# waveygang/wfmash

Measured on AMD Instinct MI355X. Metric: aligned bases/sec (whole node) + CIGAR-identical rate vs CPU ref, higher is better.
Workload: dtype int32; 1 GPU; C3: 64 synthetic 5%-divergence 50kb segment pairs per GPU, WFA-only (BiWFA gap-affine-2p 5,8,2,24,1; mappings pre-supplied); pairs_per_gpu=64, pairs_total=64, parallelism=records sharded over 1 GPU(s)

## Files before the change

wfmash_amd/csrc/wfa_device.h:

```cpp
#ifndef WFM_WFA_DEVICE_H_
#define WFM_WFA_DEVICE_H_

#include <hip/hip_runtime.h>
#include <stdint.h>

#include "wfa_rows.h"

namespace wfm {

constexpr int WF_NULL = -(1 << 30);
constexpr int RING = 32;
constexpr int RMASK = RING - 1;
constexpr int RING_BIG = 128;

enum { C_M = 0, C_I1 = 1, C_I2 = 2, C_D1 = 3, C_D2 = 4 };
enum { OP_M = 0, OP_X = 1, OP_I = 2, OP_D = 3 };
enum { BT_I1_EXT = 8, BT_I2_EXT = 16, BT_D1_EXT = 32, BT_D2_EXT = 64 };

constexpr int WFM_DEV_UNREACHABLE = -300;
constexpr int WFM_DEV_OVERFLOW = -2;
constexpr int WFM_DEV_BAND = -4;
constexpr int WFM_DEV_P2_NOTHING = -6;
constexpr int WFM_DEV_LIMIT = -7;
constexpr int WFM_DEV_P2_MORE = -5;
// ... 79 lines not shown
  int32_t score, score_fwd, score_rev, k_fwd, off_fwd, comp;
  int32_t steps;
  uint64_t cells;
  int32_t steps_p1;
  uint32_t ticks_p1, ticks_p2;
  int32_t pad_;
  uint32_t ticks_list, ticks_pick;
  uint32_t work_items, pad2_;
};

struct BaseJob {
  int64_t p_off, t_off;
  int64_t pre_off;
  int64_t bt_off;
  int64_t ring_off;
  int64_t rle_end;
  int32_t pl, tl;
  int32_t comp_begin, comp_end;
  int32_t endsfree, pbf, pef, tbf, tef;
  int32_t smax, kmin, width;
  int32_t type;
  int32_t pad_;
  int32_t score_only;
};
static_assert(sizeof(BaseJob) == 112, "BaseJob::score_only fills the struct's tail padding: the job arrays keep their stride");

struct BaseResult {
  int32_t status;
  int32_t score;
  int32_t nruns;
  int32_t pad_;
  uint64_t cells;
};

struct Base2TJob {
  BaseJob b;
  int64_t snap_in, snap_out;
  int32_t ntiles, core;
  int32_t task0;
  int32_t s0;
  int32_t done;
  int32_t end_s, end_k, end_off;
};
struct Base2TTask { int32_t job, tile; };
constexpr int B2T_ROWS = 32;
constexpr int B2T_THREADS = 512;
void launch_base2t_block(const uint32_t* pk, int32_t* a32, uint8_t* a8, const Base2TJob* jobs, const Base2TTask* tasks, unsigned long long* tile_key,
                         int32_t* tile_off, int ntasks, int T, hipStream_t st);
void launch_base2t_advance(Base2TJob* jobs, const unsigned long long* tile_key, const int32_t* tile_off, int njobs, int T, int32_t* active_slot, hipStream_t st);
void launch_base2t_finish(const int32_t* a32, const uint8_t* a8, uint32_t* rle, const Base2TJob* jobs, BaseResult* res, int njobs, hipStream_t st);

struct BoundJob { int64_t p_off, t_off; int32_t pl, tl; };
void launch_bound(const uint8_t* seq, const BoundJob* jobs, int32_t* out, int njobs, DevPen pen, hipStream_t st);

struct SeqRev { int64_t p_fwd, p_rev, t_fwd, t_rev; int32_t plen, tlen; };
void launch_reverse(uint8_t* seq, const SeqRev* jobs, int njobs, int pad, hipStream_t st);
struct SeqGatherTask { const uint8_t* src; uint8_t* dst; int32_t len, pad; int32_t reverse, complement; };
void launch_seq_gather(const SeqGatherTask* tasks, int64_t ntasks, hipStream_t st);
struct CheckProb {
  int64_t p_off, t_off;
  uint64_t run_off;
  uint32_t n_runs;
  int32_t plen, tlen;
  int32_t pbf, pef, tbf, tef;
  int32_t res_score;
  uint32_t res_ops_len;
  int32_t skip;
};
struct CheckTask { int32_t prob, slice; };
void launch_check(const uint8_t* seq, const uint32_t* runs, const CheckProb* probs, int nprob, const CheckTask* tasks, int64_t ntasks,
                  uint32_t* ops_pre, uint32_t* p_pre, uint32_t* t_pre, uint32_t* cmp_ops, unsigned long long* keys, void* out, DevPen pen,
                  hipStream_t st);
struct OptProb {
  int64_t p_off, t_off, row_off;
  int32_t plen, tlen;
  int32_t pbf, pef, tbf, tef;
  int32_t band_lo, band_hi;
};
void launch_optcheck(const uint8_t* seq, const OptProb* probs, int nprob, int form, int32_t* rows, int32_t* out, DevPen pen, hipStream_t st);
void launch_seq_normalize(uint8_t* seq, int64_t nbytes, hipStream_t st);
void launch_seq_pack(const uint8_t* seq, uint32_t* pk, int64_t nwords, int64_t nbytes, const SeqRev* jobs, int njobs, int32_t* flag, hipStream_t st);
constexpr int64_t PK_PAD_WORDS = 2048 + 64;
void launch_tile2(const uint32_t* pk, int32_t* ring, const TileJob* jobs, const TileTask* tasks, int32_t* mak, int ntasks, int threads, int T, int variants, hipStream_t st);
bool tile2_coarse_maxima();
void launch_tile2_p2(const uint32_t* pk, int32_t* ring, const TileJob* jobs, const TileTask* tasks, int ntasks, int threads, int32_t* p2, hipStream_t st);
int selftest_dpp(int* host_out128, hipStream_t st);
void launch_base2(const uint32_t* pk, int32_t* a32, uint8_t* a8, uint32_t* rle, const BaseJob* jobs, BaseResult* res, int njobs, int threads, hipStream_t st);
void launch_bp(const uint8_t* seq, int32_t* ring, const BpJob* jobs, BpResult* res, int njobs, int threads,
               DevPen pen, int scope, int ring_rows, hipStream_t st);
void launch_tile_init(const uint8_t* seq, int32_t* ring, const TileJob* jobs, int32_t* mak0, int njobs, int ring_rows, hipStream_t st);
void launch_tile(const uint8_t* seq, int32_t* ring, const TileJob* jobs, const TileTask* tasks, int32_t* mak, int ntasks,
                 int threads, int T, int Wt, size_t lds_bytes, DevPen pen, int scope, int ring_rows, hipStream_t st);
void launch_tile_advance(TileJob* jobs, int32_t* mak, int njobs, int T, DevPen pen, int exact, int coarse, int launched, hipStream_t st);
void launch_tile_reg(const uint8_t* seq, int32_t* ring, const TileJob* jobs, const TileTask* tasks, int32_t* mak, int ntasks,
                     int threads, int T, int C, bool cut, hipStream_t st);
void launch_tile_p2(const uint8_t* seq, int32_t* ring, const TileJob* jobs, const TileTask* tasks, int ntasks, int threads,
                    int32_t* p2, bool cut, hipStream_t st);
void launch_p2_to_ring(int32_t* ring, const int32_t* p2, const P2Job* jobs, int njobs, hipStream_t st);
struct RingWidenJob {
  const int32_t* src;
  int32_t* dst;
  int32_t src_w, src_koff;
  int32_t dst_w, dst_koff;
  int32_t klo, khi;
};
void launch_ring_widen(const RingWidenJob* jobs, int njobs, int max_dst_w, int ring_rows, hipStream_t st);
void launch_p2_blockmax(const int32_t* ring, const int32_t* p2, const P2Job* jobs, int32_t* bmax, int32_t* p2max, int njobs, hipStream_t st);
void launch_p2_overlap(const int32_t* ring, const int32_t* p2, const P2Job* jobs, const int32_t* p2max, const int32_t* bmax, int32_t* pbmax,
                       BpResult* res, int njobs, int threads, int max_nblk, DevPen pen, int scope, hipStream_t st);
void launch_base(const uint8_t* seq, int32_t* a32, uint8_t* a8, uint32_t* rle, const BaseJob* jobs, BaseResult* res,
                 int njobs, DevPen pen, bool wide, int ring_rows, hipStream_t st);
void launch_compact(const uint32_t* rle, const int64_t* off, const int64_t* cap, uint32_t* out, unsigned long long* total,
                    int64_t* out_start, int32_t* out_count, int nprob, hipStream_t st);

}
#endif
```

wfmash_amd/csrc/wfa_host.hip:

```cpp
#include <hip/hip_runtime.h>

#include <algorithm>
#include <chrono>
#include <climits>
#include <cstdio>
#include <cstring>
#include <atomic>
#include <mutex>
#include <string>
#include <thread>
#include <vector>

#include "../../include/wfmash_hip.h"
#include "wfa_device.h"
#include "dev_cache.h"
#include "wfa_plan.h"
#include "wfa_optband.h"

#ifdef WFM_PROFILE_SECTIONS
namespace wfm { void read_sections(long long* out); }
#endif
namespace wfm { void p2_counters(unsigned long long* out); }
namespace {

// ... 467 lines not shown
    }
    if (r.status == WFM_DEV_OVERFLOW && nd.limit > 0 && nd.smax >= nd.limit) {
      c.prob_status[nd.prob] = WFM_ST_MAX_SCORE; continue;
    }
    if (r.status == WFM_DEV_OVERFLOW) {
      if (c.pflags) c.pflags[nd.prob] |= nd.tries == 0 ? WFM_PF_BASE_RETRY : WFM_PF_BASE_RETRY2;
      Node again = nd;
      again.tries = nd.tries + 1;
      const bool constrained = nd.cb != C_M || nd.ce != C_M;
      const int64_t bound = constrained
          ? (int64_t)2 * std::max(pen.o1, pen.o2) + (int64_t)std::max(pen.e1, pen.e2) * ((int64_t)nd.pl + nd.tl) + 8
          : (int64_t)gapcost(pen, nd.pl) + gapcost(pen, nd.tl) + 8;
      if (nd.smax >= bound) {
        if (c.cfg.debug) fprintf(stderr, "[wfm] problem %d: base job pl %d tl %d cb %d ce %d overflowed its score bound %d\n", nd.prob, nd.pl, nd.tl, nd.cb, nd.ce, nd.smax);
        c.prob_status[nd.prob] = WFM_ST_UNREACHABLE; continue;
      }
      again.smax = (int32_t)std::min<int64_t>((int64_t)nd.smax * 8 + 32, bound);
      const bool to_tiles = c.rules.base_v2 && c.rules.base_tiles && is_acgt(c.S, nd.prob);
      if (nd.smax < 1020 && again.smax > 1020 && !to_tiles) again.smax = 1020;
      if (nd.limit > 0) again.smax = std::min(again.smax, nd.limit);
      c.retry.push_back(again);
    } else if (r.status != 0) {
      if (c.cfg.debug) fprintf(stderr, "[wfm] problem %d: base job pl %d tl %d status %d\n", nd.prob, nd.pl, nd.tl, r.status);
      c.prob_status[nd.prob] = WFM_ST_UNREACHABLE;
    }
  }
}

int run_base_jobs(wfm_handle* h, wfm_seqset* S, const wfm_penalties_t& pen, const BaseCfg& cfg, std::vector<Node>& nodes,
                  std::vector<Node>& retry, std::vector<int32_t>& prob_status, std::vector<uint64_t>& prob_cells,
                  LevelTimer& tm, uint32_t* pflags, std::vector<int32_t>& prob_score) {
  if (nodes.empty()) return WFM_OK;
  BaseChunk c{h, S, pen, cfg, nodes, retry, prob_status, prob_cells, tm, pflags, prob_score,
              ring_rows_for(std::max(pen.x, std::max(pen.o1 + pen.e1, pen.o2 + pen.e2)) + 1)};
  c.rules = BaseRules{cfg.base_v2, cfg.base_tiles, cfg.force_tiles, nodes.size() < 128, nodes.size() < 128 ? 512 : 2048};
  std::stable_sort(nodes.begin(), nodes.end(), [&](const Node& a, const Node& b) { return base_kind_of(c, a) < base_kind_of(c, b); });
  for (size_t i0 = 0; i0 < nodes.size(); i0 = c.end) {
    fill_base_chunk(c, i0);
    if (c.jobs.empty()) continue;
    const int rc = run_base_chunk(c);
    if (rc != WFM_OK) return rc;
    if (cfg.debug > 1) print_base_chunk(c);
    settle_base_chunk(c);
  }
  return WFM_OK;
}


struct TileCfg {
  bool exact = true;
  int T_refine = 0;
  int chunk = 2;
  int T = 100, Wt = 1024, threads = 512;
  int min_len = 128, min_score = 64;
  bool enabled = true;
  bool reg = false;
  int C = 2;
  bool fine = true;
  int debug = 0;
  bool p2_dump_on = false;
  int p2_dump = 0;
};

TileCfg tile_cfg(const wfm_penalties_t& pen, int scope) {
  TileCfg c;
  if (const char* e = getenv("WFM_TILE")) c.enabled = atoi(e) != 0;
  if (const char* e = getenv("WFM_TILE_T")) c.T = atoi(e);
  if (const char* e = getenv("WFM_TILE_T_REFINE")) c.T_refine = atoi(e);
  if (const char* e = getenv("WFM_TILE_EXACT")) c.exact = atoi(e) != 0;
  if (const char* e = getenv("WFM_TILE_W")) c.Wt = atoi(e);
  if (const char* e = getenv("WFM_TILE_THREADS")) c.threads = atoi(e);
  if (const char* e = getenv("WFM_TILE_MIN_LEN")) c.min_len = atoi(e);
  if (const char* e = getenv("WFM_TILE_MIN_SCORE")) c.min_score = atoi(e);
  c.fine = env_num("WFM_TILE_FINE", 1) != 0;
  c.debug = env_debug();
  if (const char* e = getenv("WFM_P2_DUMP")) { c.p2_dump_on = true; c.p2_dump = atoi(e); }
  const int RR = ring_rows_for(scope);
  c.T = std::max(c.T, RR);
  if (c.T_refine > 0) c.T_refine = std::max(c.T_refine, RR);
  const bool dflt = pen.x == 5 && pen.o1 + pen.e1 == 10 && pen.o2 + pen.e2 == 25 && pen.e1 == 2 && pen.e2 == 1;
  c.reg = dflt && !(getenv("WFM_TILE_REG") && atoi(getenv("WFM_TILE_REG")) == 0);
  if (c.reg) {
    if (!getenv("WFM_TILE_THREADS")) c.threads = 512;
    c.T = std::min(c.T, (int)((40 * 1024) / (4 * std::max(1, c.threads / 64))) - 1);
    if (const char* e = getenv("WFM_TILE_CHUNK")) c.chunk = std::max(1, atoi(e));
    c.Wt = c.threads * c.C;
    return c;
  }
  const size_t rows = (size_t)scope + 2 * (pen.e1 + 1) + 2 * (pen.e2 + 1);
  while ((rows * c.Wt + c.T + 1) * 4 > 160 * 1024 && c.Wt > 4 * c.T) c.Wt -= 64;
  if (c.Wt < 4 * c.T || (rows * c.Wt + c.T + 1) * 4 > 160 * 1024) c.enabled = false;
  return c;
}


inline TileJob tile_job_from(const BpJob& j) {
  TileJob t{};
  t.p_fwd = j.p_fwd; t.t_fwd = j.t_fwd; t.p_rev = j.p_rev; t.t_rev = j.t_rev;
  t.ring_in = j.ring_off;
  t.pl = j.pl; t.tl = j.tl; t.comp_begin = j.comp_begin; t.comp_end = j.comp_end;
  t.width = j.width; t.koff = j.koff; t.active = 1; t.packed = j.packed; t.sub = j.sub;
  return t;
}

struct ReuseUse { int32_t keep = 0, dir = 0, s_k = 0; };
struct ReuseCtl {
  KeepStore* store = nullptr;
  int cadence = 0;
  int slack = 0;
  int min_blocks = 1;
  std::vector<ReuseUse> use;
  std::vector<int32_t> upto;
  std::vector<int32_t> meet;
  std::vector<char> bad;
  std::vector<std::vector<int32_t>> kept[2];
  uint64_t keep_bytes = 0, restore_bytes = 0;
};

struct TilePhase {
  wfm_handle* h; wfm_seqset* S; const DevPen& dp; int scope; const TileCfg& cfg; int T; bool refine;
  std::vector<BpJob>& jobs; const std::vector<int>& tiled; std::vector<int64_t>& ring2; double& tile_ms; uint64_t& tile_cells;
  size_t n;
  std::vector<TileJob> tj, got;
  std::vector<int> fmax, rmax, s_begin;
  std::vector<char> active;
  size_t n_active = 0;
  bool any_cut = false;
  int chunk = 1;
  TilePlanRules rules;
  std::vector<TilePlanJob> pjobs;
  TileChunkPlan plan;
  uint32_t blocks = 0;
  double lane_cells = 0;
  ReuseCtl* ru = nullptr;
  std::vector<uint8_t> dirs, own;
  std::vector<int32_t> resumed_at;
  std::vector<KeepTask> ktasks;
  std::vector<int32_t> kids;
  std::vector<RestoreTask> rtasks;
  std::vector<int32_t> rres;
};

void reuse_fall_back(TilePhase& p, size_t i, bool touched = false) {
  if (p.active[i]) { p.active[i] = 0; --p.n_active; }
  p.tj[i].active = 0; p.tj[i].mode = 3;
  p.dirs[i] = 3; p.resumed_at[i] = -1;
  p.ru->bad[i] = 1;
  p.ru->store->drop(p.ru->use[i].keep);
  p.h->tile_ctr[WFM_TC_REUSE_FALLBACKS] += 1;
  p.h->tile_ctr[touched ? WFM_TC_REUSE_TOUCHED : WFM_TC_REUSE_FELL_OTHER] += 1;
}

int init_tile_jobs(TilePhase& p, const std::vector<int32_t>* fine_from, const std::vector<int64_t>* ring3) {
  wfm_handle* h = p.h;
  const TileCfg& cfg = p.cfg;
  const size_t n = p.n;
  const int T = p.T;
  p.tj.resize(n); p.fmax.assign(n, 0); p.rmax.assign(n, 0); p.active.assign(n, 1); p.s_begin.assign(n, 0);
  p.dirs.assign(n, 3); p.own.assign(n, 3); p.resumed_at.assign(n, 0);
  if (p.ru) { p.ru->bad.assign(n, 0); p.ru->kept[0].assign(n, {}); p.ru->kept[1].assign(n, {}); }
  for (size_t i = 0; i < n; ++i) {
    const BpJob& j = p.jobs[(size_t)p.tiled[i]];
    TileJob& t = p.tj[i];
    t = tile_job_from(j);
    t.ring_out = p.ring2[i];
    t.fine_s = (fine_from && i < fine_from->size()) ? (*fine_from)[i] : INT_MAX;
    t.ring_prev = (ring3 && i < ring3->size() && (*ring3)[i] >= 0 && (j.packed & 1) && cfg.reg && cfg.exact && !p.refine) ? (*ring3)[i] : -1;
// ... 2174 lines not shown
```

wfmash_amd/csrc/wfa_tile2.hip:

```cpp
#include <hip/hip_runtime.h>
#include <stdint.h>
#include <type_traits>

#include "wfa_device.h"
#include "wfa_base.h"
#include "wfa_pack.h"

#ifdef WFM_TILE_TRACE
__device__ unsigned long long g_tile_trace[48 * 16 * 128 * 4];
extern "C" int wfm_debug_tile_trace(unsigned long long* out, size_t n) {
  return (int)hipMemcpyFromSymbol(out, HIP_SYMBOL(g_tile_trace), n * sizeof(unsigned long long), 0, hipMemcpyDeviceToHost);
}
#if WFM_TILE_TRACE == 1
#define WFM_TRACE_STAMP(slot_) do { if (trace_on) { const unsigned long long ts_ = __builtin_readcyclecounter(); if (lane == 0) g_tile_trace[(((size_t)blockIdx.x * 16 + wv) * 128 + (t & 127)) * 4 + (slot_)] = ts_; } } while (0)
#else
#define WFM_TRACE_STAMP(slot_) do { } while (0)
#endif
#define WFM_TRACE_MARK(idx_) do { if (WFM_TILE_TRACE == 2 && trace_on2) { const unsigned long long ts_ = __builtin_readcyclecounter(); if (lane == 0) g_tile_trace[(((size_t)blockIdx.x * 16 + wv) * 128 + (idx_)) * 4] = ts_; } } while (0)
#else
#define WFM_TRACE_STAMP(slot_) do { } while (0)
#define WFM_TRACE_MARK(idx_) do { } while (0)
#endif

namespace wfm {
// ... 153 lines not shown
    const uint32_t x = pk16_win(SRC.lP, oP[c]) ^ pk16_win(SRC.lT, oT[c]);
    ext[c] = min((int)first_diff16(x), maxn[c]);
    R.mm[c] = __builtin_amdgcn_ballot_w64(m[c] >= 0) & __builtin_amdgcn_ballot_w64(ext[c] >= 16);
    R.outw |= m[c] > lim[c];
  }
  return R;
}
__device__ __forceinline__ void pk_rare2_fast(const PkSrc& SRC, PkProbe R, const int (&m)[2], const unsigned (&oP)[2], const unsigned (&oT)[2], const int (&maxn)[2],
                                              const int (&lim)[2], int (&ext)[2], bool tail_direct) {
  if (__builtin_expect(__any(R.outw), 0)) {
#pragma unroll
    for (int c = 0; c < 2; ++c) {
      bool more = m[c] >= 0 && ext[c] >= 16;
      if (m[c] > lim[c]) {
        const uint32_t x = pk16(SRC.gP, oP[c]) ^ pk16(SRC.gT, oT[c]);
        ext[c] = min((int)first_diff16(x), maxn[c]);
        more = ext[c] >= 16;
      }
      R.mm[c] = __builtin_amdgcn_ballot_w64(more);
    }
  }
  const unsigned lane = threadIdx.x & 63u;
#pragma unroll
  for (int c = 0; c < 2; ++c) {
    if (__builtin_expect(R.mm[c] != 0, 0)) {
      const bool more = (R.mm[c] >> lane) & 1ull;
      bool tail = false;
      if (tail_direct && __popcll(R.mm[c]) <= (unsigned)TAIL_DIRECT_MAX) tail = more;
      else if (more) {
        const int n = pk_stage2(SRC, oP[c], oT[c]);
        ext[c] = min(n, maxn[c]);
        tail = n >= 80 && maxn[c] > 80;
      }
      if (__any(tail)) ext[c] = pk_wave_tail(SRC, oP[c], oT[c], ext[c], maxn[c], tail);
    }
  }
}
__device__ __forceinline__ void pk_extend2_fast(const PkSrc& SRC, const int (&m)[2], const unsigned (&oP)[2], const unsigned (&oT)[2], const int (&maxn)[2],
                                                const int (&lim)[2], int (&ext)[2], bool tail_direct) {
  const PkProbe R = pk_probe2_fast(SRC, m, oP, oT, maxn, lim, ext);
  pk_rare2_fast(SRC, R, m, oP, oT, maxn, lim, ext, tail_direct);
}

}

__global__ __launch_bounds__(256) void seq_pack_kernel(const uint8_t* __restrict__ seq, uint32_t* __restrict__ pk, int64_t nwords, int64_t nbytes) {
  const int64_t i = (int64_t)blockIdx.x * blockDim.x + threadIdx.x;
  if (i >= nwords) return;
  uint32_t v = 0;
  if ((i + 1) * 16 <= nbytes) {
    const uint4 q = *reinterpret_cast<const uint4*>(seq + i * 16);
    const uint32_t w[4] = {q.x, q.y, q.z, q.w};
#pragma unroll
    for (int j = 0; j < 4; ++j) {
      const uint32_t c = (w[j] >> 1) & 0x03030303u;
      v |= ((c & 3u) | ((c >> 6) & 0xcu) | ((c >> 12) & 0x30u) | ((c >> 18) & 0xc0u)) << (8 * j);
    }
  } else {
    for (int j = 0; j < 16; ++j) {
      const int64_t a = i * 16 + j;
      const uint32_t c = a < nbytes ? (uint32_t)seq[a] : 0u;
      v |= pack_code((uint8_t)c) << (2 * j);
    }
  }
  pk[i] = v;
}
__global__ __launch_bounds__(256) void seq_acgt_kernel(const uint8_t* __restrict__ seq, const SeqRev* __restrict__ jobs, int32_t* __restrict__ flag) {
  const SeqRev J = jobs[blockIdx.x >> 1];
  const bool text = blockIdx.x & 1;
  const uint8_t* src = seq + (text ? J.t_fwd : J.p_fwd);
  const int n = text ? J.tlen : J.plen;
  bool bad = false;
  for (int q = threadIdx.x; q < n; q += blockDim.x) {
    const uint8_t c = src[q];
    bad |= !pack_is_acgt(c);
  }
  if (__any(bad) && (threadIdx.x & 63) == 0) flag[blockIdx.x >> 1] = 0;
}
void launch_seq_pack(const uint8_t* seq, uint32_t* pk, int64_t nwords, int64_t nbytes, const SeqRev* jobs, int njobs, int32_t* flag, hipStream_t st) {
  if (nwords > 0) hipLaunchKernelGGL(seq_pack_kernel, dim3((unsigned)((nwords + 255) / 256)), dim3(256), 0, st, seq, pk, nwords, nbytes);
  if (njobs > 0) hipLaunchKernelGGL(seq_acgt_kernel, dim3((unsigned)njobs * 2), dim3(256), 0, st, seq, jobs, flag);
}

template <int NTMAX, bool P2, bool FAST, bool FINE = true>
__global__ __launch_bounds__(NTMAX) void wfa_tile2_kernel(const uint32_t* __restrict__ pk, int32_t* __restrict__ ring_arena,
                                                        const TileJob* __restrict__ jobs, const TileTask* __restrict__ tasks,
                                                        int32_t* __restrict__ mak_out, int T, int32_t* __restrict__ p2_arena, int coarse) {
  constexpr int C = 2, LB = 25, H = LB + 1, NCL = 5, DEP = 6, E1 = 2;
  constexpr bool WAVE1 = NTMAX == 64;
  constexpr bool PIPE = FAST && !P2;
  __shared__ __attribute__((aligned(16))) int s_edge[2][WAVE1 ? 1 : 17][2][4];
  __shared__ __attribute__((aligned(16))) uint32_t s_winP[PK_WIN_DW + PK_SLACK_DW], s_winT[PK_WIN_DW + PK_SLACK_DW];
  __shared__ int s_wlo[2];
  extern __shared__ __attribute__((aligned(16))) int s_makr[];
  TileTask tk = tasks[blockIdx.x];
  const TileJob J = jobs[tk.job];
  if (!J.active) return;
  const int sbase = P2 ? (tk.dir == 0 ? J.tf : J.tr) : (J.mode == 6 ? J.s0 - T : J.s0);
  const Rng RG = make_rng(J.pl, J.tl, J.sub);
  const bool lowdiv = (J.packed & 2) != 0;
  int halo = T;
  {
    const int s1 = sbase + T;
    int L, R;
    rng_block(RG, sbase, s1, L, R);
    const int idx = tk.core_lo, core = tk.core_hi;
    tk.core_lo = L + idx * core;
    tk.core_hi = min(R, tk.core_lo + core - 1);
    if (tk.core_lo > R) return;
    if (tk.core_lo == L && tk.core_hi == R) halo = 0;
  }
  const int dir = tk.dir, tid = threadIdx.x, lane = tid & 63, wv = tid >> 6;
  const int kA = tk.core_lo - halo;
  const int nw = min((int)(blockDim.x >> 6), (tk.core_hi + halo - kA) / (64 * C) + 1), NT = nw * 64;
  if (wv >= nw) return;
#ifdef WFM_TILE_TRACE
  const bool trace_on2 = !P2 && FAST && !WAVE1 && gridDim.x >= 512 && blockIdx.x < 48 && sbase == 4000 && J.mode == 0;
#endif
  WFM_TRACE_MARK(120);
  if (tid < 2) s_wlo[tid] = INT32_MAX;
  if (!WAVE1) for (int i = tid; i < (int)(sizeof(s_edge) / sizeof(int)); i += NT) ((int*)s_edge)[i] = WF_NULL;
  const int64_t aP = dir == 0 ? J.p_fwd : J.p_rev, aT = dir == 0 ? J.t_fwd : J.t_rev;
  const int pl = J.pl, tl = J.tl, s0 = sbase;
  const int k0 = kA + tid * C;
  const int64_t width = J.width;
  const int32_t* rin = ring_arena + ((!P2 && J.mode == 6) ? J.ring_prev : J.ring_in) + J.koff + (int64_t)dir * 5 * RING * width;
  int32_t* rout = ring_arena + J.ring_out + J.koff + (int64_t)dir * 5 * RING * width;
  const int kmax = tk.core_hi + halo;
  const int Tn = (!P2 && J.mode == 1) ? (dir == 0 ? J.tf : J.tr) : T;
  const int t_stream = Tn - ((J.mode == 1 || J.mode == 6 || J.ring_prev < 0) ? H : E1);
  if (!P2 && FAST && !(coarse & 2)) {
    const bool fine = !(coarse & 1) || J.mode == 5 || (J.mode == 0 && sbase + T >= J.fine_s);
    if (fine != FINE) return;
  }
  __shared__ int s_run[(!P2 && FAST && !FINE) ? NTMAX : 1];
  if (!P2 && FAST && !FINE) s_run[tid] = 0;

  int Mh[C][NCL][DEP];
  int I1h[C][E1], D1h[C][E1], I2h[C], D2h[C];
  const bool lean_on = (coarse & 4) != 0;
  if (lean_on && tile_wave_lean_load(RG, __builtin_amdgcn_readfirstlane(k0), kmax, s0)) {
    const int32_t* const wrow = rin + __builtin_amdgcn_readfirstlane(k0);
    const unsigned lofs = (unsigned)lane * (unsigned)(C * sizeof(int32_t));
    auto ld_lean = [&](int comp, int sc, int& a, int& b) {
      ld_pair(reinterpret_cast<const int32_t*>(reinterpret_cast<const char*>(wrow + ((int64_t)(comp * RING + (sc & RMASK))) * width) + lofs), a, b);
    };
#pragma unroll
    for (int d = 0; d < H; ++d) ld_lean(C_M, s0 - d, Mh[0][(NCL - d % NCL) % NCL][d / NCL], Mh[1][(NCL - d % NCL) % NCL][d / NCL]);
#pragma unroll
    for (int r = 1; r < NCL; ++r) { Mh[0][r][DEP - 1] = WF_NULL; Mh[1][r][DEP - 1] = WF_NULL; }
#pragma unroll
    for (int d = 0; d < E1; ++d) {
      ld_lean(C_I1, s0 - d, I1h[0][d], I1h[1][d]);
      ld_lean(C_D1, s0 - d, D1h[0][d], D1h[1][d]);
    }
    ld_lean(C_I2, s0, I2h[0], I2h[1]);
    ld_lean(C_D2, s0, D2h[0], D2h[1]);
  } else {
    __builtin_amdgcn_s_waitcnt(0x0F70);
    const bool kin0 = k0 <= kmax, kin1 = k0 + 1 <= kmax;
#pragma unroll
    for (int c = 0; c < C; ++c)
#pragma unroll
      for (int r = 0; r < NCL; ++r)
#pragma unroll
        for (int e = 0; e < DEP; ++e) Mh[c][r][e] = WF_NULL;
    auto ld_row = [&](int comp, int sc, int& a, int& b) {
      const int lo = rng_lo(RG, sc), hi = rng_hi(RG, sc);
      const bool ok0 = kin0 && sc >= 0 && k0 >= lo && k0 <= hi, ok1 = kin1 && sc >= 0 && k0 + 1 >= lo && k0 + 1 <= hi;
      int x = WF_NULL, y = WF_NULL;
      if (ok0 || ok1) ld_pair(rin + ((int64_t)(comp * RING + (sc & RMASK))) * width + k0, x, y);
      a = ok0 ? x : WF_NULL; b = ok1 ? y : WF_NULL;
    };
#pragma unroll
    for (int d = 0; d < H; ++d)
      ld_row(C_M, s0 - d, Mh[0][(NCL - d % NCL) % NCL][d / NCL], Mh[1][(NCL - d % NCL) % NCL][d / NCL]);
#pragma unroll
    for (int d = 0; d < E1; ++d) {
      ld_row(C_I1, s0 - d, I1h[0][d], I1h[1][d]);
      ld_row(C_D1, s0 - d, D1h[0][d], D1h[1][d]);
    }
    ld_row(C_I2, s0, I2h[0], I2h[1]);
    ld_row(C_D2, s0, D2h[0], D2h[1]);
  }
  const int MKS = T + 1;
  if (FINE && !P2) for (int t = tid; t < (FAST && !WAVE1 ? nw * MKS : MKS); t += NT) s_makr[t] = 0;
  unsigned hmaxu[C];
  int s_last[C];
  int negk[C];
  bool incore[C];
#pragma unroll
  for (int c = 0; c < C; ++c) {
    const int k = k0 + c;
    const bool colok = (k >= -pl) && (k <= tl);
    hmaxu[c] = colok ? (unsigned)min(tl, pl + k) : 0u;
    s_last[c] = colok ? min(k - RG.kb_lo, RG.kb_hi - k) : -1;
    incore[c] = k >= tk.core_lo && k <= tk.core_hi;
    negk[c] = incore[c] ? -k : -(1 << 29);
  }
  {
    int hlo = INT32_MAX, vlo = INT32_MAX;
#pragma unroll
    for (int c = 0; c < C; ++c) {
      const int k = k0 + c;
      int lo = INT32_MAX;
#pragma unroll
      for (int r = 0; r < NCL; ++r)
#pragma unroll
        for (int e = 0; e < DEP; ++e) lo = min(lo, Mh[c][r][e] >= 0 ? Mh[c][r][e] : INT32_MAX);
#pragma unroll
      for (int d = 0; d < E1; ++d) { lo = min(lo, I1h[c][d] >= 0 ? I1h[c][d] : INT32_MAX); lo = min(lo, D1h[c][d] >= 0 ? D1h[c][d] : INT32_MAX); }
      lo = min(lo, I2h[c] >= 0 ? I2h[c] : INT32_MAX);
      lo = min(lo, D2h[c] >= 0 ? D2h[c] : INT32_MAX);
      if (lo != INT32_MAX) { hlo = min(hlo, lo); vlo = min(vlo, lo - k); }
    }
    WFM_TRACE_MARK(124);
    __syncthreads();
    if (hlo != INT32_MAX) { atomicMin(&s_wlo[0], hlo); atomicMin(&s_wlo[1], max(vlo, 0)); }
    __syncthreads();
  }
  WFM_TRACE_MARK(125);
  const int wT0 = s_wlo[0] == INT32_MAX ? 0 : s_wlo[0], wP0 = s_wlo[1] == INT32_MAX ? 0 : s_wlo[1];
  const int64_t oriP = (aP + wP0) & ~(int64_t)15, oriT = (aT + wT0) & ~(int64_t)15;
  const int dP = (int)(aP - oriP), dT = (int)(aT - oriT);
  PkSrc SRC;
  SRC.lP = (lds_words)s_winP; SRC.lT = (lds_words)s_winT;
  SRC.gP = (glb_words)pk + (oriP >> 4); SRC.gT = (glb_words)pk + (oriT >> 4);
  for (int i = tid; i < PK_WIN_DW + PK_SLACK_DW; i += NT) {
    s_winP[i] = SRC.gP[i];
    s_winT[i] = SRC.gT[i];
  }
  int cP[C];
  int wlim[C];
#pragma unroll
  for (int c = 0; c < C; ++c) { cP[c] = dP - (k0 + c); wlim[c] = PK_WIN_BASES - 1 - max(cP[c], dT); }
  __syncthreads();

  constexpr int UB = FAST ? 2 * NCL : NCL;
  int pM[C];
  if (PIPE) {
#pragma unroll
    for (int c = 0; c < C; ++c) {
      pM[c] = Mh[c][0][0];
      const int l1 = Mh[c][0][1], l2 = Mh[c][0][2], l3 = Mh[c][0][3], l4 = Mh[c][0][4], l5 = Mh[c][0][5];
      Mh[c][0][DEP - 1] = l1; Mh[c][0][0] = l2; Mh[c][0][1] = l3; Mh[c][0][2] = l4; Mh[c][0][3] = l5;
    }
  }
  constexpr int EDGE_PLANE = (WAVE1 ? 1 : 17) * 2 * 4;
  const bool edge_lane = lane == 0 || lane == 63;
  int* const edge_wr = lane == 63 ? &s_edge[0][WAVE1 ? 0 : wv + 1][0][0] : &s_edge[0][WAVE1 ? 0 : wv][1][0];
  auto stream_gap_rows = [&](int s, const int (&vI1)[C], const int (&vI2)[C], const int (&vD1)[C], const int (&vD2)[C]) {
#pragma unroll
    for (int c = 0; c < C; ++c) {
      if (incore[c] && s <= s_last[c]) {
        const int64_t ro = ((int64_t)(s & RMASK)) * width + k0 + c;
        rout[(int64_t)C_I1 * RING * width + ro] = vI1[c];
        rout[(int64_t)C_I2 * RING * width + ro] = vI2[c];
        rout[(int64_t)C_D1 * RING * width + ro] = vD1[c];
        rout[(int64_t)C_D2 * RING * width + ro] = vD2[c];
      }
    }
  };
  auto line_take = [&](auto JJX, const int (&row)[C]) {
    constexpr int jjx = decltype(JJX)::value;
    constexpr int clx = jjx % NCL;
#pragma unroll
    for (int c = 0; c < C; ++c) {
      if (jjx <= NCL) Mh[c][clx][DEP - 1] = row[c];
      else {
// ... 56 lines not shown
      lM10 = from_prev_lane0(M_S10(C - 1)); lM25 = from_prev_lane0(M_S25(C - 1));
      lI1 = from_prev_lane0(I1h[C - 1][e1x]); lI2 = from_prev_lane0(I2h[C - 1]);
      rM10 = from_next_lane0(M_S10(0)); rM25 = from_next_lane0(M_S25(0));
      rD1 = from_next_lane0(D1h[0][e1x]); rD2 = from_next_lane0(D2h[0]);
      if (lane == 0)  { const int* e = s_edge[par][wv][0];     lM10 = e[0]; lM25 = e[1]; lI1 = e[2]; lI2 = e[3]; }
      if (lane == 63) { const int* e = s_edge[par][wv + 1][1]; rM10 = e[0]; rM25 = e[1]; rD1 = e[2]; rD2 = e[3]; }
      }
    } else {
      lM10 = from_prev_lane(M_S10(C - 1)); lM25 = from_prev_lane(M_S25(C - 1));
      lI1 = from_prev_lane(I1h[C - 1][e1x]); lI2 = from_prev_lane(I2h[C - 1]);
      rM10 = from_next_lane(M_S10(0)); rM25 = from_next_lane(M_S25(0));
      rD1 = from_next_lane(D1h[0][e1x]); rD2 = from_next_lane(D2h[0]);
    }
    int nM[C], nI1[C], nI2[C], nD1[C], nD2[C], nMis[C];
    int pext[C], pmaxn[C];
    unsigned poP[C], poT[C];
    PkProbe PR;
    if (PIPE) {
#pragma unroll
      for (int c = 0; c < C; ++c) { poP[c] = (unsigned)(pM[c] + cP[c]); poT[c] = (unsigned)(pM[c] + dT); pmaxn[c] = (int)hmaxu[c] - pM[c]; }
      PR = pk_probe2_fast(SRC, pM, poP, poT, pmaxn, wlim, pext);
    }
#pragma unroll
    for (int c = 0; c < C; ++c) {
      const int a10 = c == 0 ? lM10 : M_S10(c - 1), b10 = c == C - 1 ? rM10 : M_S10(c + 1);
      const int a25 = c == 0 ? lM25 : M_S25(c - 1), b25 = c == C - 1 ? rM25 : M_S25(c + 1);
      const int i1 = c == 0 ? lI1 : I1h[c - 1][e1x], d1 = c == C - 1 ? rD1 : D1h[c + 1][e1x];
      const int i2 = c == 0 ? lI2 : I2h[c - 1], d2 = c == C - 1 ? rD2 : D2h[c + 1];
      const int mx = M_S5(c);
      const unsigned hm = hmaxu[c];
      int ins1 = max(a10, i1) + 1, ins2 = max(a25, i2) + 1, del1 = max(b10, d1), del2 = max(b25, d2), mis = mx + 1;
      if (!FAST) {
        ins1 = (unsigned)ins1 <= hm ? ins1 : WF_NULL;
        ins2 = (unsigned)ins2 <= hm ? ins2 : WF_NULL;
        del1 = (unsigned)del1 <= hm ? del1 : WF_NULL;
        del2 = (unsigned)del2 <= hm ? del2 : WF_NULL;
        mis = (unsigned)mis <= hm ? mis : WF_NULL;
      }
      nI1[c] = ins1; nI2[c] = ins2; nD1[c] = del1; nD2[c] = del2; nMis[c] = mis;
      nM[c] = max(max(max(ins1, ins2), mis), max(del1, del2));
    }
    if (FAST) {
      bool special = false;
#pragma unroll
      for (int c = 0; c < C; ++c) special |= (nM[c] > (int)hmaxu[c]) | (s > s_last[c]);
      if (__builtin_expect(__any(special), 0)) {
#pragma unroll
        for (int c = 0; c < C; ++c) {
          const unsigned hm = hmaxu[c];
          nI1[c] = (unsigned)nI1[c] <= hm ? nI1[c] : WF_NULL;
          nI2[c] = (unsigned)nI2[c] <= hm ? nI2[c] : WF_NULL;
          nD1[c] = (unsigned)nD1[c] <= hm ? nD1[c] : WF_NULL;
          nD2[c] = (unsigned)nD2[c] <= hm ? nD2[c] : WF_NULL;
          const int mis = (unsigned)nMis[c] <= hm ? nMis[c] : WF_NULL;
          nM[c] = max(max(max(nI1[c], nI2[c]), mis), max(nD1[c], nD2[c]));
          nM[c] = s <= s_last[c] ? nM[c] : WF_NULL;
        }
      }
    } else {
#pragma unroll
      for (int c = 0; c < C; ++c) nM[c] = s <= s_last[c] ? nM[c] : WF_NULL;
    }
    if (PIPE) {
      pk_rare2_fast(SRC, PR, pM, poP, poT, pmaxn, wlim, pext, lowdiv);
      int fin[C], mak = 0;
#pragma unroll
      for (int c = 0; c < C; ++c) {
        fin[c] = pM[c] + pext[c];
        mak = max(mak, pM[c] >= 0 ? 2 * fin[c] + negk[c] : 0);
      }
      switch (jj) {
        case 1: line_take(std::integral_constant<int, UB>{}, fin); break;
        case 2: line_take(std::integral_constant<int, 1>{}, fin); break;
        case 3: line_take(std::integral_constant<int, 2>{}, fin); break;
        case 4: line_take(std::integral_constant<int, 3>{}, fin); break;
        case 5: line_take(std::integral_constant<int, 4>{}, fin); break;
        case 6: line_take(std::integral_constant<int, 5>{}, fin); break;
        case 7: line_take(std::integral_constant<int, 6>{}, fin); break;
        case 8: line_take(std::integral_constant<int, 7>{}, fin); break;
        case 9: line_take(std::integral_constant<int, 8>{}, fin); break;
        default: line_take(std::integral_constant<int, 9>{}, fin); break;
      }
      if (!FINE) (void)__hip_atomic_fetch_max(&s_run[tid], mak, __ATOMIC_RELAXED, __HIP_MEMORY_SCOPE_WORKGROUP);
      else {
        mak = wave_max63(mak);
        if (lane == 63) s_makr[(WAVE1 ? 0 : wv * MKS) + t - 1] = mak;
      }
      if (__builtin_expect(t > t_stream, 0)) {
        stream_gap_rows(s, nI1, nI2, nD1, nD2);
      }
#pragma unroll
      for (int c = 0; c < C; ++c) { pM[c] = nM[c]; I1h[c][e1x] = nI1[c]; D1h[c][e1x] = nD1[c]; I2h[c] = nI2[c]; D2h[c] = nD2[c]; }
    } else {
    int ext[C], maxn[C];
    unsigned oP[C], oT[C];
#pragma unroll
    for (int c = 0; c < C; ++c) {
      const int m = nM[c];
      oP[c] = (unsigned)(m + cP[c]); oT[c] = (unsigned)(m + dT);
      maxn[c] = (FAST || m >= 0) ? (int)hmaxu[c] - m : 0;
    }
    WFM_TRACE_STAMP(1);
    if (FAST) pk_extend2_fast(SRC, nM, oP, oT, maxn, wlim, ext, lowdiv);
    else pk_extend2<false>(SRC, nM, oP, oT, maxn, ext, lowdiv);
#ifdef WFM_TILE_TRACE
    if (trace_on) asm volatile("" :: "v"(ext[0]), "v"(ext[1]));
#endif
    WFM_TRACE_STAMP(2);
    int mak = 0;
#pragma unroll
    for (int c = 0; c < C; ++c) {
      const int m = nM[c];
      const int me = m + ext[c];
      const bool live = m >= 0;
      nM[c] = (FAST || live) ? me : WF_NULL;
      mak = max(mak, live ? 2 * me + negk[c] : 0);
    }
    if (P2) {
      int32_t* prow = p2_arena + J.p2_off + J.koff2 + ((int64_t)(dir * 5) * P2K + (t - 1)) * J.w2;
      const int64_t cstride = (int64_t)P2K * J.w2;
      const bool w0 = incore[0] && s <= s_last[0], w1 = incore[1] && s <= s_last[1];
      if (w0 && w1) {
        st_pair(prow + C_M * cstride + k0, nM[0], nM[1]); st_pair(prow + C_I1 * cstride + k0, nI1[0], nI1[1]); st_pair(prow + C_I2 * cstride + k0, nI2[0], nI2[1]);
        st_pair(prow + C_D1 * cstride + k0, nD1[0], nD1[1]); st_pair(prow + C_D2 * cstride + k0, nD2[0], nD2[1]);
      } else {
#pragma unroll
        for (int c = 0; c < C; ++c) {
          const int k = k0 + c;
          if (c == 0 ? w0 : w1) {
            prow[C_M * cstride + k] = nM[c]; prow[C_I1 * cstride + k] = nI1[c]; prow[C_I2 * cstride + k] = nI2[c];
            prow[C_D1 * cstride + k] = nD1[c]; prow[C_D2 * cstride + k] = nD2[c];
          }
        }
      }
    }
    if (!P2 && __builtin_expect(t > t_stream, 0)) {
      stream_gap_rows(s, nI1, nI2, nD1, nD2);
    }
#pragma unroll
    for (int c = 0; c < C; ++c) {
      if (!FAST) {
#pragma unroll
        for (int e = DEP - 1; e > 0; --e) Mh[c][cl][e] = Mh[c][cl][e - 1];
        Mh[c][cl][0] = nM[c];
#pragma unroll
        for (int d = E1 - 1; d > 0; --d) { I1h[c][d] = I1h[c][d - 1]; D1h[c][d] = D1h[c][d - 1]; }
        I1h[c][0] = nI1[c]; D1h[c][0] = nD1[c];
      } else {
        if (!vB) Mh[c][cl][DEP - 1] = nM[c];
        else {
          const int parked = Mh[c][cl][DEP - 1];
#pragma unroll
          for (int e = DEP - 1; e > 1; --e) Mh[c][cl][e] = Mh[c][cl][e - 2];
          Mh[c][cl][1] = parked;
          Mh[c][cl][0] = nM[c];
        }
        I1h[c][e1x] = nI1[c]; D1h[c][e1x] = nD1[c];
      }
      I2h[c] = nI2[c]; D2h[c] = nD2[c];
    }
    if (!P2) {
      if (FAST && !FINE) (void)__hip_atomic_fetch_max(&s_run[tid], mak, __ATOMIC_RELAXED, __HIP_MEMORY_SCOPE_WORKGROUP);
      else {
        mak = wave_max63(mak);
        if (FAST) { if (lane == 63) s_makr[(WAVE1 ? 0 : wv * MKS) + t] = mak; }
        else if (lane == 63 && mak > 0) {
          if (WAVE1) s_makr[t] = mak;
          else atomicMax(&s_makr[t], mak);
        }
      }
    }
    }
#undef M_S5
#undef M_S10
#undef M_S25
  }
  }
  if (PIPE) {
    int pext[C], pmaxn[C], fin[C], mak = 0;
    unsigned poP[C], poT[C];
#pragma unroll
    for (int c = 0; c < C; ++c) { poP[c] = (unsigned)(pM[c] + cP[c]); poT[c] = (unsigned)(pM[c] + dT); pmaxn[c] = (int)hmaxu[c] - pM[c]; }
    pk_extend2_fast(SRC, pM, poP, poT, pmaxn, wlim, pext, lowdiv);
#pragma unroll
    for (int c = 0; c < C; ++c) {
      fin[c] = pM[c] + pext[c];
      mak = max(mak, pM[c] >= 0 ? 2 * fin[c] + negk[c] : 0);
    }
    switch (Tn % UB) {
      case 1: line_take(std::integral_constant<int, 1>{}, fin); break;
      case 2: line_take(std::integral_constant<int, 2>{}, fin); break;
      case 3: line_take(std::integral_constant<int, 3>{}, fin); break;
      case 4: line_take(std::integral_constant<int, 4>{}, fin); break;
      case 5: line_take(std::integral_constant<int, 5>{}, fin); break;
      case 6: line_take(std::integral_constant<int, 6>{}, fin); break;
      case 7: line_take(std::integral_constant<int, 7>{}, fin); break;
      case 8: line_take(std::integral_constant<int, 8>{}, fin); break;
      case 9: line_take(std::integral_constant<int, 9>{}, fin); break;
      default: line_take(std::integral_constant<int, UB>{}, fin); break;
    }
    if (!FINE) (void)__hip_atomic_fetch_max(&s_run[tid], mak, __ATOMIC_RELAXED, __HIP_MEMORY_SCOPE_WORKGROUP);
    else { mak = wave_max63(mak); if (lane == 63) s_makr[(WAVE1 ? 0 : wv * MKS) + Tn] = mak; }
  }
  WFM_TRACE_MARK(122);
  if (P2) return;
  if (FAST) {
    const int r10 = Tn % UB;
#pragma unroll
    for (int j0 = 1; j0 <= NCL; ++j0) {
      if (r10 >= j0 && r10 < j0 + NCL) {
        const int clx = j0 % NCL;
#pragma unroll
        for (int c = 0; c < C; ++c) {
          const int parked = Mh[c][clx][DEP - 1];
#pragma unroll
          for (int e = DEP - 1; e > 0; --e) Mh[c][clx][e] = Mh[c][clx][e - 1];
          Mh[c][clx][0] = parked;
        }
      }
    }
  }
  const int s_end = s0 + Tn;
  if (Tn < H) {
#pragma unroll
    for (int c = 0; c < C; ++c) {
      const int k = k0 + c;
      if (!incore[c]) continue;
      for (int d = Tn; d < H; ++d) {
        const int sc = s_end - d;
        if (sc < 0 || k < rng_lo(RG, sc) || k > rng_hi(RG, sc)) continue;
        const int64_t ro = ((int64_t)(sc & RMASK)) * width + k;
        rout[(int64_t)C_I1 * RING * width + ro] = rin[(int64_t)C_I1 * RING * width + ro];
        rout[(int64_t)C_I2 * RING * width + ro] = rin[(int64_t)C_I2 * RING * width + ro];
        rout[(int64_t)C_D1 * RING * width + ro] = rin[(int64_t)C_D1 * RING * width + ro];
        rout[(int64_t)C_D2 * RING * width + ro] = rin[(int64_t)C_D2 * RING * width + ro];
      }
    }
  }
  const int k0w = __builtin_amdgcn_readfirstlane(k0);
  const bool lean_st = (coarse & 4) != 0 && tile_wave_lean_store(RG, k0w, tk.core_lo, tk.core_hi, s_end, Tn);
  int32_t* const wrow_out = rout + k0w;
  const unsigned lofs_out = (unsigned)lane * (unsigned)(C * sizeof(int32_t));
  auto write_rows = [&](auto TR) {
    constexpr int tr = decltype(TR)::value;
    if (lean_st) {
      if (incore[0])
#pragma unroll
      for (int d = 0; d < H; ++d) {
        const int r = ((tr - d) % NCL + NCL) % NCL, back = ((tr - r) % NCL + NCL) % NCL, e = (d - back) / NCL;
        char* const row = reinterpret_cast<char*>(wrow_out + ((int64_t)(C_M * RING + ((s_end - d) & RMASK))) * width);
        st_pair(reinterpret_cast<int32_t*>(row + lofs_out), Mh[0][r][e], Mh[1][r][e]);
      }
      return;
    }
    if (!incore[0] && !incore[1]) return;
#pragma unroll
    for (int d = 0; d < H; ++d) {
      constexpr int dummy = 0; (void)dummy;
      const int r = ((tr - d) % NCL + NCL) % NCL;
      const int back = ((tr - r) % NCL + NCL) % NCL;
      const int e = (d - back) / NCL;
      const int sc = s_end - d;
      const int lo = rng_lo(RG, sc), hi = rng_hi(RG, sc);
      const bool w0 = incore[0] && sc >= 0 && k0 >= lo && k0 <= hi, w1 = incore[1] && sc >= 0 && k0 + 1 >= lo && k0 + 1 <= hi;
      int32_t* dst = rout + ((int64_t)(C_M * RING + (sc & RMASK))) * width + k0;
      if (w0 && w1) st_pair(dst, Mh[0][r][e], Mh[1][r][e]);
      else {
        if (w0) dst[0] = Mh[0][r][e];
        if (w1) dst[1] = Mh[1][r][e];
      }
    }
  };
  switch (Tn % NCL) {
    case 0: write_rows(std::integral_constant<int, 0>{}); break;
    case 1: write_rows(std::integral_constant<int, 1>{}); break;
    case 2: write_rows(std::integral_constant<int, 2>{}); break;
    case 3: write_rows(std::integral_constant<int, 3>{}); break;
    default: write_rows(std::integral_constant<int, 4>{}); break;
  }
  int32_t* mk = mak_out + ((int64_t)tk.job * 2 + dir) * T;
  WFM_TRACE_MARK(123);
  if (!FINE) {
    if (J.mode == 0) {
      const int makrun = wave_max63(s_run[tid]);
      if (lane == 63 && makrun > 0) atomicMax(&mk[T - 1], makrun);
    }
    return;
  }
  __syncthreads();
  for (int t = 1 + tid; t <= T; t += NT) {
    int v = s_makr[t];
    if (FAST && !WAVE1) for (int w = 1; w < nw; ++w) v = max(v, s_makr[w * MKS + t]);
    if (v > 0) atomicMax(&mk[t - 1], v);
  }
}

static bool tile_fast() {
  const char* e = getenv("WFM_TILE_FAST");
  return !(e && atoi(e) == 0);
}
static int tile_lean() {
  const char* e = getenv("WFM_TILE_LEAN");
  return (e && atoi(e) == 0) ? 0 : 4;
}
bool tile2_coarse_maxima() {
  const char* e = getenv("WFM_TILE_COARSE");
  return tile_fast() && !(e && atoi(e) == 0);
}
void launch_tile2(const uint32_t* pk, int32_t* ring, const TileJob* jobs, const TileTask* tasks, int32_t* mak, int ntasks, int threads, int T,
                  int variants, hipStream_t st) {
  const size_t lds1 = (size_t)(T + 1) * 4;
  const int lean = tile_lean();
  if (tile_fast()) {
    const int coarse = tile2_coarse_maxima() ? 1 : 0;
    if (!coarse) variants = 2;
    const size_t pad = getenv("WFM_TILE_LDS_PAD") ? (size_t)atoi(getenv("WFM_TILE_LDS_PAD")) : 0;
    if (variants & 1) {
      if (threads <= 64) hipLaunchKernelGGL((wfa_tile2_kernel<64, false, true, false>), dim3(ntasks), dim3(64), 0, st, pk, ring, jobs, tasks, mak, T, (int32_t*)nullptr, coarse | lean);
      else hipLaunchKernelGGL((wfa_tile2_kernel<1024, false, true, false>), dim3(ntasks), dim3(threads), pad, st, pk, ring, jobs, tasks, mak, T, (int32_t*)nullptr, coarse | lean);
    }
    if (variants & 2) {
      const int cf = coarse | (variants == 2 ? 2 : 0);
      if (threads <= 64) hipLaunchKernelGGL((wfa_tile2_kernel<64, false, true, true>), dim3(ntasks), dim3(64), lds1, st, pk, ring, jobs, tasks, mak, T, (int32_t*)nullptr, cf | lean);
      else hipLaunchKernelGGL((wfa_tile2_kernel<1024, false, true, true>), dim3(ntasks), dim3(threads), lds1 * (size_t)(threads / 64), st, pk, ring, jobs, tasks, mak, T, (int32_t*)nullptr, cf | lean);
    }
  } else {
    if (threads <= 64) hipLaunchKernelGGL((wfa_tile2_kernel<64, false, false, true>), dim3(ntasks), dim3(64), lds1, st, pk, ring, jobs, tasks, mak, T, (int32_t*)nullptr, lean);
    else hipLaunchKernelGGL((wfa_tile2_kernel<1024, false, false, true>), dim3(ntasks), dim3(threads), lds1, st, pk, ring, jobs, tasks, mak, T, (int32_t*)nullptr, lean);
  }
}
void launch_tile2_p2(const uint32_t* pk, int32_t* ring, const TileJob* jobs, const TileTask* tasks, int ntasks, int threads, int32_t* p2, hipStream_t st) {
  const size_t lds1 = (size_t)(P2K + 1) * 4;
  const int lean = tile_lean();
  if (tile_fast()) {
    if (threads <= 64) hipLaunchKernelGGL((wfa_tile2_kernel<64, true, true, false>), dim3(ntasks), dim3(64), 0, st, pk, ring, jobs, tasks, (int32_t*)nullptr, P2K, p2, lean);
    else hipLaunchKernelGGL((wfa_tile2_kernel<1024, true, true, false>), dim3(ntasks), dim3(threads), 0, st, pk, ring, jobs, tasks, (int32_t*)nullptr, P2K, p2, lean);
  } else {
    if (threads <= 64) hipLaunchKernelGGL((wfa_tile2_kernel<64, true, false, true>), dim3(ntasks), dim3(64), lds1, st, pk, ring, jobs, tasks, (int32_t*)nullptr, P2K, p2, lean);
    else hipLaunchKernelGGL((wfa_tile2_kernel<1024, true, false, true>), dim3(ntasks), dim3(threads), lds1, st, pk, ring, jobs, tasks, (int32_t*)nullptr, P2K, p2, lean);
  }
}

constexpr int B2_C = 2, B2_NCL = 5, B2_DEP = 6, B2_E1 = 2;
constexpr DevPen B2_PEN{5, 8, 2, 24, 1};

__device__ __forceinline__ PkSrc b2_load_windows(const BaseJob& J, const uint32_t* __restrict__ pk, uint32_t* s_winP, uint32_t* s_winT, int tid, int stride,
                                                 int& dP, int& dT) {
  const int64_t oriP = J.p_off & ~(int64_t)15, oriT = J.t_off & ~(int64_t)15;
  dP = (int)(J.p_off - oriP); dT = (int)(J.t_off - oriT);
  PkSrc SRC;
  SRC.lP = (lds_words)s_winP; SRC.lT = (lds_words)s_winT;
  SRC.gP = (glb_words)pk + (oriP >> 4); SRC.gT = (glb_words)pk + (oriT >> 4);
  const int nP = min(PK_WIN_DW + PK_SLACK_DW, (J.pl + dP + 15) / 16 + 8), nT = min(PK_WIN_DW + PK_SLACK_DW, (J.tl + dT + 15) / 16 + 8);
  for (int i = tid; i < nP; i += stride) s_winP[i] = SRC.gP[i];
  for (int i = tid; i < nT; i += stride) s_winT[i] = SRC.gT[i];
  return SRC;
}

__device__ __forceinline__ void b2_end_checks(const BaseJob& J, int* s_done, int* s_endk, int k, int m_ext, int ins1, int ins2, int del1, int del2) {
  const int pl = J.pl, tl = J.tl;
  if (J.endsfree) {
    if (m_ext >= 0) {
      const int h = m_ext, v = m_ext - k;
      if ((h >= tl && pl - v <= J.pef) || (v >= pl && tl - h <= J.tef)) atomicMin(s_endk, k);
    }
  } else if (k == tl - pl) {
    const int ev = J.comp_end == C_M ? m_ext : (J.comp_end == C_I1 ? ins1 : (J.comp_end == C_I2 ? ins2 : (J.comp_end == C_D1 ? del1 : del2)));
    if (ev >= tl) *s_done = 1;
  }
}

__device__ __forceinline__ void b2_row0(const BaseJob& J, const PkSrc& SRC, int dT, int lo0, int hi0, int k0, const int (&cP)[B2_C], const bool (&keep)[B2_C],
                                        int32_t* pre_base, uint8_t* bt_base, int* s_done, int* s_endk, int (&Mh)[B2_C][B2_NCL][B2_DEP], int (&I1h)[B2_C][B2_E1],
                                        int (&D1h)[B2_C][B2_E1], int (&I2h)[B2_C], int (&D2h)[B2_C], int (&mcur)[B2_C]) {
  constexpr int C = B2_C;
  const int pl = J.pl, tl = J.tl, k_end = tl - pl;
  int m0[C], ext[C], maxn[C];
  unsigned oP[C], oT[C];
#pragma unroll
  for (int c = 0; c < C; ++c) {
    const int k = k0 + c;
    const bool on = k >= lo0 && k <= hi0;
    int m = WF_NULL;
    if (on) {
      if (J.endsfree) m = k > 0 ? k : 0;
      else {
        if (J.comp_begin == C_M) m = 0;
        I1h[c][0] = J.comp_begin == C_I1 ? 0 : WF_NULL;
        I2h[c] = J.comp_begin == C_I2 ? 0 : WF_NULL;
        D1h[c][0] = J.comp_begin == C_D1 ? 0 : WF_NULL;
        D2h[c] = J.comp_begin == C_D2 ? 0 : WF_NULL;
      }
    }
    m0[c] = m;
    oP[c] = (unsigned)(m + cP[c]); oT[c] = (unsigned)(m + dT);
    maxn[c] = m >= 0 ? min(pl - (m - k), tl - m) : 0;
  }
  pk_extend2(SRC, m0, oP, oT, maxn, ext);
#pragma unroll
  for (int c = 0; c < C; ++c) {
    const int k = k0 + c;
    if (k < lo0 || k > hi0) continue;
    if (keep[c]) { pre_base[k] = m0[c]; bt_base[k] = 0; }
    int m = m0[c];
    if (m >= 0) m += ext[c];
    if (keep[c]) {
      if (J.endsfree) b2_end_checks(J, s_done, s_endk, k, m, WF_NULL, WF_NULL, WF_NULL, WF_NULL);
// ... 474 lines not shown
```

Baseline: 58.68 million aligned bases/s.

## Replace per-wave max reductions with slotted LDS atomic maxima in tile2 kernel

```diff
diff --git a/wfmash_amd/csrc/wfa_device.h b/wfmash_amd/csrc/wfa_device.h
--- a/wfmash_amd/csrc/wfa_device.h
+++ b/wfmash_amd/csrc/wfa_device.h
@@ -185,6 +185,11 @@
 void launch_seq_pack(const uint8_t* seq, uint32_t* pk, int64_t nwords, int64_t nbytes, const SeqRev* jobs, int njobs, int32_t* flag, hipStream_t st);
 constexpr int64_t PK_PAD_WORDS = 2048 + 64;
 void launch_tile2(const uint32_t* pk, int32_t* ring, const TileJob* jobs, const TileTask* tasks, int32_t* mak, int ntasks, int threads, int T, int variants, hipStream_t st);
+#ifndef WFM_TILE_SLOTS_WIDE
+#define WFM_TILE_SLOTS_WIDE 16
+#endif
+constexpr int TILE_SLOTS_WAVE1 = 2, TILE_SLOTS_SMALL = 4, TILE_SLOTS_WIDE = WFM_TILE_SLOTS_WIDE;
+constexpr int tile_fine_slots(int threads) { return threads <= 64 ? TILE_SLOTS_WAVE1 : (threads <= 128 ? TILE_SLOTS_SMALL : TILE_SLOTS_WIDE); }
 bool tile2_coarse_maxima();
 void launch_tile2_p2(const uint32_t* pk, int32_t* ring, const TileJob* jobs, const TileTask* tasks, int ntasks, int threads, int32_t* p2, hipStream_t st);
 int selftest_dpp(int* host_out128, hipStream_t st);
diff --git a/wfmash_amd/csrc/wfa_host.hip b/wfmash_amd/csrc/wfa_host.hip
--- a/wfmash_amd/csrc/wfa_host.hip
+++ b/wfmash_amd/csrc/wfa_host.hip
@@ -573,7 +573,8 @@
   c.reg = dflt && !(getenv("WFM_TILE_REG") && atoi(getenv("WFM_TILE_REG")) == 0);
   if (c.reg) {
     if (!getenv("WFM_TILE_THREADS")) c.threads = 512;
-    c.T = std::min(c.T, (int)((40 * 1024) / (4 * std::max(1, c.threads / 64))) - 1);
+    c.T = std::min(c.T, (int)((40 * 1024) / (4 * TILE_SLOTS_WIDE)) - 1);
+    while (c.threads * c.C <= 2 * c.T && c.threads < 1024) c.threads += 64;
     if (const char* e = getenv("WFM_TILE_CHUNK")) c.chunk = std::max(1, atoi(e));
     c.Wt = c.threads * c.C;
     return c;
diff --git a/wfmash_amd/csrc/wfa_tile2.hip b/wfmash_amd/csrc/wfa_tile2.hip
--- a/wfmash_amd/csrc/wfa_tile2.hip
+++ b/wfmash_amd/csrc/wfa_tile2.hip
@@ -259,13 +259,15 @@
   if (njobs > 0) hipLaunchKernelGGL(seq_acgt_kernel, dim3((unsigned)njobs * 2), dim3(256), 0, st, seq, jobs, flag);
 }
 
-template <int NTMAX, bool P2, bool FAST, bool FINE = true>
+template <int NTMAX, bool P2, bool FAST, bool FINE = true, int MS = 0>
 __global__ __launch_bounds__(NTMAX) void wfa_tile2_kernel(const uint32_t* __restrict__ pk, int32_t* __restrict__ ring_arena,
                                                         const TileJob* __restrict__ jobs, const TileTask* __restrict__ tasks,
                                                         int32_t* __restrict__ mak_out, int T, int32_t* __restrict__ p2_arena, int coarse) {
   constexpr int C = 2, LB = 25, H = LB + 1, NCL = 5, DEP = 6, E1 = 2;
   constexpr bool WAVE1 = NTMAX == 64;
   constexpr bool PIPE = FAST && !P2;
+  constexpr bool SLOTS = FAST && FINE && !P2;
+  static_assert(!SLOTS || (MS >= 2 && MS <= 64 && (MS & (MS - 1)) == 0), "slots per score: a power of two within a wave");
   __shared__ __attribute__((aligned(16))) int s_edge[2][WAVE1 ? 1 : 17][2][4];
   __shared__ __attribute__((aligned(16))) uint32_t s_winP[PK_WIN_DW + PK_SLACK_DW], s_winT[PK_WIN_DW + PK_SLACK_DW];
   __shared__ int s_wlo[2];
@@ -360,8 +362,11 @@
     ld_row(C_I2, s0, I2h[0], I2h[1]);
     ld_row(C_D2, s0, D2h[0], D2h[1]);
   }
-  const int MKS = T + 1;
-  if (FINE && !P2) for (int t = tid; t < (FAST && !WAVE1 ? nw * MKS : MKS); t += NT) s_makr[t] = 0;
+  if (FINE && !P2) for (int t = tid; t < (SLOTS ? (T + 1) * MS : T + 1); t += NT) s_makr[t] = 0;
+  unsigned mk_off = (unsigned)(lane & (MS - 1)) * 4u;
+  auto slot_max = [&](int j, int mak) {
+    (void)__hip_atomic_fetch_max(static_cast<int*>(__builtin_assume_aligned(reinterpret_cast<char*>(s_makr) + mk_off, 4)) + j * MS, mak, __ATOMIC_RELAXED, __HIP_MEMORY_SCOPE_WORKGROUP);
+  };
   unsigned hmaxu[C];
   int s_last[C];
   int negk[C];
@@ -584,10 +589,7 @@
         default: line_take(std::integral_constant<int, 9>{}, fin); break;
       }
       if (!FINE) (void)__hip_atomic_fetch_max(&s_run[tid], mak, __ATOMIC_RELAXED, __HIP_MEMORY_SCOPE_WORKGROUP);
-      else {
-        mak = wave_max63(mak);
-        if (lane == 63) s_makr[(WAVE1 ? 0 : wv * MKS) + t - 1] = mak;
-      }
+      else slot_max(jj - 1, mak);
       if (__builtin_expect(t > t_stream, 0)) {
         stream_gap_rows(s, nI1, nI2, nD1, nD2);
       }
@@ -665,8 +667,7 @@
       if (FAST && !FINE) (void)__hip_atomic_fetch_max(&s_run[tid], mak, __ATOMIC_RELAXED, __HIP_MEMORY_SCOPE_WORKGROUP);
       else {
         mak = wave_max63(mak);
-        if (FAST) { if (lane == 63) s_makr[(WAVE1 ? 0 : wv * MKS) + t] = mak; }
-        else if (lane == 63 && mak > 0) {
+        if (lane == 63 && mak > 0) {
           if (WAVE1) s_makr[t] = mak;
           else atomicMax(&s_makr[t], mak);
         }
@@ -677,6 +678,7 @@
 #undef M_S10
 #undef M_S25
   }
+    if (SLOTS) { mk_off += (unsigned)(UB * MS * 4); asm volatile("" : "+v"(mk_off)); }
   }
   if (PIPE) {
     int pext[C], pmaxn[C], fin[C], mak = 0;
@@ -702,7 +704,7 @@
       default: line_take(std::integral_constant<int, UB>{}, fin); break;
     }
     if (!FINE) (void)__hip_atomic_fetch_max(&s_run[tid], mak, __ATOMIC_RELAXED, __HIP_MEMORY_SCOPE_WORKGROUP);
-    else { mak = wave_max63(mak); if (lane == 63) s_makr[(WAVE1 ? 0 : wv * MKS) + Tn] = mak; }
+    else slot_max(Tn - (Tn + UB - 1) / UB * UB, mak);
   }
   WFM_TRACE_MARK(122);
   if (P2) return;
@@ -790,11 +792,17 @@
     return;
   }
   __syncthreads();
-  for (int t = 1 + tid; t <= T; t += NT) {
-    int v = s_makr[t];
-    if (FAST && !WAVE1) for (int w = 1; w < nw; ++w) v = max(v, s_makr[w * MKS + t]);
-    if (v > 0) atomicMax(&mk[t - 1], v);
-  }
+  if (SLOTS) {
+    for (int i0 = wv * 64; i0 < T * MS; i0 += NT) {
+      const int i = i0 + lane;
+      int v = i < T * MS ? s_makr[MS + i] : 0;
+#pragma unroll
+      for (int o = MS / 2; o > 0; o >>= 1) v = max(v, __shfl_xor(v, o));
+      if ((i & (MS - 1)) == 0 && i < T * MS && v > 0) atomicMax(&mk[i / MS], v);
+    }
+    return;
+  }
+  for (int t = 1 + tid; t <= T; t += NT) if (s_makr[t] > 0) atomicMax(&mk[t - 1], s_makr[t]);
 }
 
 static bool tile_fast() {
@@ -823,8 +831,10 @@
     }
     if (variants & 2) {
       const int cf = coarse | (variants == 2 ? 2 : 0);
-      if (threads <= 64) hipLaunchKernelGGL((wfa_tile2_kernel<64, false, true, true>), dim3(ntasks), dim3(64), lds1, st, pk, ring, jobs, tasks, mak, T, (int32_t*)nullptr, cf | lean);
-      else hipLaunchKernelGGL((wfa_tile2_kernel<1024, false, true, true>), dim3(ntasks), dim3(threads), lds1 * (size_t)(threads / 64), st, pk, ring, jobs, tasks, mak, T, (int32_t*)nullptr, cf | lean);
+      const size_t ldsm = lds1 * (size_t)tile_fine_slots(threads);
+      if (threads <= 64) hipLaunchKernelGGL((wfa_tile2_kernel<64, false, true, true, TILE_SLOTS_WAVE1>), dim3(ntasks), dim3(64), ldsm, st, pk, ring, jobs, tasks, mak, T, (int32_t*)nullptr, cf | lean);
+      else if (threads <= 128) hipLaunchKernelGGL((wfa_tile2_kernel<1024, false, true, true, TILE_SLOTS_SMALL>), dim3(ntasks), dim3(threads), ldsm, st, pk, ring, jobs, tasks, mak, T, (int32_t*)nullptr, cf | lean);
+      else hipLaunchKernelGGL((wfa_tile2_kernel<1024, false, true, true, TILE_SLOTS_WIDE>), dim3(ntasks), dim3(threads), ldsm, st, pk, ring, jobs, tasks, mak, T, (int32_t*)nullptr, cf | lean);
     }
   } else {
     if (threads <= 64) hipLaunchKernelGGL((wfa_tile2_kernel<64, false, false, true>), dim3(ntasks), dim3(64), lds1, st, pk, ring, jobs, tasks, mak, T, (int32_t*)nullptr, lean);
```

Result: faster. 60.15 million aligned bases/s, median of 6 (+2.5%).
